# openpsi-project/srl

Hardware: AMD Instinct MI355X
Metric: env-steps/sec through GAE+PPO update, 4096 envs x 128 steps (higher is better)
Workload: dtype f32 (contractions as bf16x3 / f16x2 piece products, float32 accumulate)

## Files before the change

srl_amd/csrc/h2conv.h:

```cpp
#pragma once
#include "h2gemm.h"

namespace srlh2 {

typedef float h2_f32x4 __attribute__((ext_vector_type(4)));

enum { H2C_F2 = 0, H2C_F3 = 1, H2C_D3 = 2, H2C_D2 = 3 };
enum { H2S_LINEAR = 0, H2S_PLANAR = 1, H2S_ROWS = 2, H2S_ROWSWZ = 3 };
enum { H2D_PLANAR = 0, H2D_ROWS = 1, H2D_F32_ROUTED = 2 };

template <int ID> struct H2Geo;

template <> struct H2Geo<H2C_F2> {
  static constexpr int CGW = 1;
  static constexpr int CB = 1, NCH = 64, NTAP = 16, GW = 10, OH = 9, OW = 9, NPIX_L = 400, G = 1, PLANE_E = 400;
  static constexpr int SRC = H2S_ROWSWZ, PAD = 0, SH = 20, SW = 20, SPIX = 400;
  static constexpr int DST = H2D_PLANAR, OPIX = 81, OCH = 64;
  static constexpr bool ZERO_BORDER = false;
  static constexpr bool DENSE = false;
  __host__ __device__ static constexpr int tap_u(int t) { return (((t >> 2) & 1) * 2 + (t & 1)) * 100 + (t >> 3) * 10 + ((t & 3) >> 1); }
  __host__ __device__ static constexpr int tap_k(int t) { return t; }
};
template <> struct H2Geo<H2C_F3> {
  static constexpr int CGW = 1;
  static constexpr int CB = 2, NCH = 64, NTAP = 9, GW = 9, OH = 7, OW = 7, NPIX_L = 81, G = 2, PLANE_E = 176;
  static constexpr int SRC = H2S_PLANAR, PAD = 0, SH = 9, SW = 9, SPIX = 81;
  static constexpr int DST = H2D_ROWS, OPIX = 49, OCH = 64;
  static constexpr bool ZERO_BORDER = false;
  static constexpr bool DENSE = false;
  __host__ __device__ static constexpr int tap_u(int t) { return (t / 3) * 9 + t % 3; }
  __host__ __device__ static constexpr int tap_k(int t) { return t; }
};
template <> struct H2Geo<H2C_D3> {
  static constexpr int CGW = 1;
  static constexpr int CB = 2, NCH = 64, NTAP = 9, GW = 11, OH = 9, OW = 9, NPIX_L = 121, G = 2, PLANE_E = 256;
  static constexpr int SRC = H2S_ROWS, PAD = 2, SH = 7, SW = 7, SPIX = 49;
  static constexpr int DST = H2D_PLANAR, OPIX = 81, OCH = 64;
  static constexpr bool ZERO_BORDER = true;
  static constexpr bool DENSE = true;
  __host__ __device__ static constexpr int tap_u(int t) { return (2 - t / 3) * 11 + (2 - t % 3); }
  __host__ __device__ static constexpr int tap_k(int t) { return t; }
};
template <> struct H2Geo<H2C_D2> {
  static constexpr int CGW = 2;
  static constexpr int CB = 2, NCH = 128, NTAP = 4, GW = 11, OH = 10, OW = 10, NPIX_L = 121, G = 2, PLANE_E = 256;
  static constexpr int SRC = H2S_PLANAR, PAD = 1, SH = 9, SW = 9, SPIX = 81;
  static constexpr int DST = H2D_F32_ROUTED, OPIX = 400, OCH = 32;
  static constexpr bool ZERO_BORDER = true;
  static constexpr bool DENSE = true;
  __host__ __device__ static constexpr int tap_u(int t) { return (1 - t / 2) * 11 + (1 - t % 2); }
  __host__ __device__ static constexpr int tap_k(int t) { return t; }
};

struct H2ConvArgs {
  const void* x;
  const void* w;
  const float* sx;
  const float* sw;
  int64_t n;
  const float* bias;
  int32_t act;
  void* out;
  float* out_scale;
  const float* bound_in;
  const float* bound_w;
  const float* bound_b;
  float* out_absmax;
  uint8_t* mask_out;
  const void* mask_in;
};

#ifdef __HIPCC__

template <int ID> constexpr int h2c_src_img_bytes() { return H2Geo<ID>::SPIX * H2Geo<ID>::CB * 128; }
template <int ID> constexpr int h2c_slot_bytes() { return H2Geo<ID>::CB * 8 * H2Geo<ID>::PLANE_E * 16; }

__device__ __forceinline__ uint32_t h2_xor32(uint32_t x, bool upper) {
#if __has_builtin(__builtin_amdgcn_permlane32_swap)
  typedef unsigned h2_u32x2 __attribute__((ext_vector_type(2)));
  const h2_u32x2 r = __builtin_amdgcn_permlane32_swap(x, x, false, false);
  return upper ? r[0] : r[1];
#else
  (void)upper;
  return (uint32_t)__shfl_xor((int)x, 32);
#endif
}

#ifndef SRL_H2C_SCHED
#define SRL_H2C_SCHED 1
#endif

template <int NKB> struct H2ActiveKb { int n; int kb[NKB]; };
template <int RM, int NTAP, int CB, int TPR> constexpr H2ActiveKb<NTAP * CB> h2_active_kbs() {
  H2ActiveKb<NTAP * CB> a{};
  for (int kb = 0; kb < NTAP * CB; ++kb)
    if ((RM >> ((kb / CB) / TPR)) & 1) a.kb[a.n++] = kb;
  return a;
}

template <int ID, int NSLOT>
__global__ __launch_bounds__(512, 2) void h2conv_kernel(H2ConvArgs a) {
  using GE = H2Geo<ID>;
  constexpr int CB = GE::CB, NKB = GE::NTAP * CB, NPL = CB * 8, PLANE_B = GE::PLANE_E * 16;
  constexpr int SLOT = NPL * PLANE_B;
  constexpr int NCG = GE::NCH / 16;
  constexpr int CGW = GE::CGW, NWG = NCG / CGW;
  constexpr int NPH = 8 / NWG;
  static_assert(NWG == 4 || NWG == 8, "");
  constexpr int NE = GE::DENSE ? GE::OH * GE::OW : (GE::OH - 1) * GE::GW + GE::OW;
  constexpr int NB_IMG = (NE + 15) / 16;
  constexpr int NBT = NB_IMG * GE::G;
  static_assert(NBT % NPH == 0 && NPH <= 2, "blocks split evenly over the (at most two) position halves");
  constexpr int NDMA = SLOT / 1024;
  constexpr int NDW = (NDMA + 7) / 8;
  static_assert(SLOT % 1024 == 0, "");
  constexpr int KROW = NKB * 128;
  constexpr int IMGB = h2c_src_img_bytes<ID>();
  constexpr bool ROUTED = GE::DST == H2D_F32_ROUTED;
  constexpr int OIMGB = GE::OPIX * GE::OCH * 4;
  constexpr int MIMGB = GE::OPIX * GE::OCH / 8;
  constexpr bool MASK_IN = ID == H2C_D3 || ID == H2C_D2, MASK_OUT = !MASK_IN;
  constexpr int MREG = MASK_IN ? (GE::G * MIMGB + 1023) / 1024 * 1024 : 0;
  constexpr int SLOTM = SLOT + MREG;
  constexpr int NDM = MREG / 1024;
  extern __shared__ __attribute__((aligned(1024))) uint8_t lds[];

  const int tid = threadIdx.x, lane = tid & 63;
  const int wid = __builtin_amdgcn_readfirstlane(tid >> 6);
  const int cg0 = (wid % NWG) * CGW, ph = wid / NWG;
  const int p = lane & 15, quad = lane >> 4;
  const bool up = quad >> 1;

  h2_f16x8 wf[CGW][NKB][2];
  {
#pragma unroll
    for (int c = 0; c < CGW; ++c) {
      const uint8_t* wr = static_cast<const uint8_t*>(a.w) + (size_t)((cg0 + c) * 16 + p) * KROW + quad * 32;
#pragma unroll
      for (int kb = 0; kb < NKB; ++kb) {
        wf[c][kb][0] = *reinterpret_cast<const h2_f16x8*>(wr + kb * 128);
        wf[c][kb][1] = *reinterpret_cast<const h2_f16x8*>(wr + kb * 128 + 16);
      }
    }
#pragma unroll
    for (int c = 0; c < CGW; ++c)
#pragma unroll
      for (int kb = 0; kb < NKB; ++kb) asm volatile("" : "+v"(wf[c][kb][0]), "+v"(wf[c][kb][1]));
  }
  const float inv = 1.f / (*a.sx * *a.sw);
  float oscale = 1.f;
  if (!ROUTED) {
    float bound = *a.bound_in * *a.bound_w;
    if (a.bound_b) bound += *a.bound_b;
    oscale = h2_scale_for(bound);
    if (blockIdx.x == 0 && tid == 0) *a.out_scale = oscale;
  }
  float bq[CGW][4];
#pragma unroll
  for (int c = 0; c < CGW; ++c) {
    bq[c][0] = bq[c][1] = bq[c][2] = bq[c][3] = 0.f;
    if (a.bias) {
      const float4 b4 = *reinterpret_cast<const float4*>(a.bias + (cg0 + c) * 16 + 4 * quad);
      bq[c][0] = b4.x; bq[c][1] = b4.y; bq[c][2] = b4.z; bq[c][3] = b4.w;
    }
  }
  const float lo = a.act == 1 ? 0.f : -3.0e38f;

  if (GE::ZERO_BORDER) {
    for (int i = tid; i < NSLOT * SLOTM / 16; i += 512) reinterpret_cast<uint4*>(lds)[i] = make_uint4(0, 0, 0, 0);
    __syncthreads();
  }

  const h2_i32x4 rx = h2_rsrc(a.x);
  h2_i32x4 rmd = h2_rsrc(MASK_IN ? a.mask_in : a.x);
  rmd[2] = MASK_IN ? (int)(a.n * MIMGB) : 0;
  const uint32_t lds0 = (uint32_t)(uintptr_t)(__attribute__((address_space(3))) uint8_t*)lds;
  const long nbatch = (a.n + GE::G - 1) / GE::G;

  uint32_t dvoff[NDW];
  int dimg[NDW];
#pragma unroll
  for (int q = 0; q < NDW; ++q) {
    const int j = wid + 8 * q;
    const int nent = j * 64 + lane;
    if (GE::SRC == H2S_LINEAR) {
      dvoff[q] = (uint32_t)(nent * 16);
      dimg[q] = j < NDMA ? 0 : -1;
    } else if (GE::SRC == H2S_ROWSWZ) {
      const int P = nent >> 3, sl = nent & 7;
      dvoff[q] = (uint32_t)(P * 128 + 16 * (sl ^ (((P >> 1) & 1) | (((P >> 2) & 1) << 2))));
      dimg[q] = j < NDMA ? 0 : -1;
    } else {
      const int plane = nent / GE::PLANE_E, e = nent - plane * GE::PLANE_E;
      const int il = e / GE::NPIX_L, cell = e - il * GE::NPIX_L;
      const int gy = cell / GE::GW, gx = cell - gy * GE::GW;
      const int sy = gy - GE::PAD, sx = gx - GE::PAD;
      const bool ok = j < NDMA && il < GE::G && (unsigned)sy < (unsigned)GE::SH && (unsigned)sx < (unsigned)GE::SW;
      const int sp = sy * GE::SW + sx;
      if (GE::SRC == H2S_PLANAR) dvoff[q] = (uint32_t)(il * IMGB + plane * (GE::SPIX * 16) + sp * 16);
      else dvoff[q] = (uint32_t)((il * GE::SPIX + sp) * (CB * 128) + plane * 16);
      dimg[q] = ok ? il : -1;
      if (!ok) dvoff[q] = 0;
    }
  }
  auto issue = [&](long b, int s) {
    const long img0 = b * GE::G;
    const int left = (int)(a.n - img0 < GE::G ? a.n - img0 : GE::G);
    const uint32_t soff = __builtin_amdgcn_readfirstlane((uint32_t)(img0 * (long)IMGB));
#pragma unroll
    for (int q = 0; q < NDW; ++q) {
      const uint32_t ldsa = __builtin_amdgcn_readfirstlane(lds0 + s * SLOTM + (wid + 8 * q) * 1024);
      if (dimg[q] >= 0 && dimg[q] < left)
        asm volatile("s_mov_b32 m0, %0\n\ts_nop 4\n\tbuffer_load_dwordx4 %1, %2, %3 offen lds" ::"s"(ldsa), "v"(dvoff[q]), "s"(rx), "s"(soff) : "memory");
    }
    if (MASK_IN && wid < NDM) {
      const uint32_t ldsa = __builtin_amdgcn_readfirstlane(lds0 + s * SLOTM + SLOT + wid * 1024);
      const uint32_t msoff = __builtin_amdgcn_readfirstlane((uint32_t)(img0 * (long)MIMGB));
      const uint32_t mvoff = (uint32_t)(wid * 1024 + lane * 16);
      asm volatile("s_mov_b32 m0, %0\n\ts_nop 4\n\tbuffer_load_dwordx4 %1, %2, %3 offen lds" ::"s"(ldsa), "v"(mvoff), "s"(rmd), "s"(msoff) : "memory");
    }
  };

  uint32_t lane_out[CGW];
  uint32_t lane_mout[CGW];
  int mi_shift[CGW], mi_pix[CGW];
  int pix_step_y, pix_step_x;
#pragma unroll
  for (int c = 0; c < CGW; ++c) {
    const int cg = cg0 + c;
    const int g_out = 2 * (quad & 1) + (cg & 1), ocb = cg >> 1;
    if (ROUTED) {
      const int cls = cg >> 1, py = cls >> 1, px = cls & 1;
      lane_out[c] = (uint32_t)(((py * 20 + px) * GE::OCH + 16 * (cg & 1) + 4 * quad) * 4);
      lane_mout[c] = 0;
      mi_shift[c] = 16 * (cg & 1) + 4 * quad;
      mi_pix[c] = py * 20 + px;
    } else {
      lane_out[c] = GE::DST == H2D_PLANAR ? (uint32_t)((((ocb * 4 + g_out) * 2 + (up ? 1 : 0)) * GE::OPIX) * 16)
                                          : (uint32_t)(ocb * 128 + g_out * 32 + (up ? 16 : 0));
      lane_mout[c] = (uint32_t)(ocb * 4 + g_out);
      mi_shift[c] = 0;
      mi_pix[c] = 0;
    }
  }
  if (ROUTED) { pix_step_y = 40; pix_step_x = 2; }
  else { pix_step_y = GE::OW; pix_step_x = 1; }
  constexpr int PIXB = ROUTED ? GE::OCH * 4 : (GE::DST == H2D_PLANAR ? 16 : GE::OCH * 4);
  const uint32_t lane_base = GE::SRC == H2S_ROWSWZ ? (uint32_t)(p * 128 + quad * 32) : (uint32_t)(quad * 2 * PLANE_B + p * 16);
  int swz_d0[8], swz_d1[8];
  if (GE::SRC == H2S_ROWSWZ) {
    static_assert(GE::SRC != H2S_ROWSWZ || SLOTM % 128 == 0, "slot stride must keep address bits 4-6");
    const uint32_t a_ref = (uint32_t)(uintptr_t)(lds + lane_base);
#pragma unroll
    for (int u = 0; u < 8; ++u) {
      const int k = (p + u) & 7;
      const uint32_t x = (uint32_t)((((k >> 1) & 1) | (((k >> 2) & 1) << 2)) * 16);
      swz_d0[u] = u * 128 + (int)((a_ref ^ x) - a_ref);
      swz_d1[u] = u * 128 + (int)((a_ref ^ x ^ 16u) - a_ref);
    }
  }
  float amax = 0.f;

  struct Meta {
    uint32_t pixoff;
    bool ok;
    long img;
    uint32_t bits[CGW];
  };
  const __amdgpu_buffer_rsrc_t r_out = __builtin_amdgcn_make_buffer_rsrc(a.out, 0, (int)(a.n * OIMGB), 0x00020000);
  const __amdgpu_buffer_rsrc_t r_mo = __builtin_amdgcn_make_buffer_rsrc(MASK_OUT ? (void*)a.mask_out : a.out, 0, (int)(a.n * MIMGB), 0x00020000);
  constexpr uint32_t OOB = 0x80000000u;
  auto epilogue1 = [&](const h2_f32x4& acc, const Meta& m, const float (&bqc)[4], uint32_t lane_out_c, uint32_t lane_mout_c, uint32_t mbits) {
    float v[4];
    constexpr bool CLAMP = ID == H2C_F2 || ID == H2C_F3;
#pragma unroll
    for (int r = 0; r < 4; ++r) v[r] = CLAMP ? fmaxf(acc[r] * inv + bqc[r], lo) : acc[r] * inv + bqc[r];
    const bool ok = m.ok;
    const uint32_t img32 = (uint32_t)m.img;
    if (MASK_IN) {
#pragma unroll
      for (int r = 0; r < 4; ++r) v[r] = __uint_as_float(__float_as_uint(v[r]) & (uint32_t)__builtin_amdgcn_sbfe((int)mbits, r, 1));
    }
    {
      const float m3 = __builtin_fmaxf(__builtin_fmaxf(fabsf(v[0]), fabsf(v[1])), fabsf(v[2]));
      const float m5 = __builtin_fmaxf(__builtin_fmaxf(m3, fabsf(v[3])), amax);
      amax = m.ok ? m5 : amax;
    }
    const uint32_t ooff = ok ? m.pixoff * PIXB + lane_out_c : OOB;
    typedef uint32_t h2_u32x4 __attribute__((ext_vector_type(4)));
    if (ROUTED) {
      h2_u32x4 d = {__float_as_uint(v[0]), __float_as_uint(v[1]), __float_as_uint(v[2]), __float_as_uint(v[3])};
      __builtin_amdgcn_raw_buffer_store_b128(d, r_out, ooff + img32 * (uint32_t)OIMGB, 0, 0);
    } else {
      uint32_t h0a, h0b, h1a, h1b;
      h2_split_pair(v[0], v[1], oscale, h0a, h1a);
      h2_split_pair(v[2], v[3], oscale, h0b, h1b);
      h2_u32x4 chunk;
#if __has_builtin(__builtin_amdgcn_permlane32_swap)
      typedef unsigned h2_u32x2 __attribute__((ext_vector_type(2)));
      const h2_u32x2 sa = __builtin_amdgcn_permlane32_swap(h0a, h1a, false, false);
      const h2_u32x2 sb = __builtin_amdgcn_permlane32_swap(h0b, h1b, false, false);
      chunk[0] = sa[0]; chunk[1] = sb[0]; chunk[2] = sa[1]; chunk[3] = sb[1];
#else
      const uint32_t r0 = h2_xor32(up ? h0a : h1a, up), r1 = h2_xor32(up ? h0b : h1b, up);
      chunk[0] = up ? r0 : h0a; chunk[1] = up ? r1 : h0b; chunk[2] = up ? h1a : r0; chunk[3] = up ? h1b : r1;
#endif
      __builtin_amdgcn_raw_buffer_store_b128(chunk, r_out, ooff + img32 * (uint32_t)OIMGB, 0, 0);
      if (MASK_OUT) {
        uint32_t nib = (v[0] > 0.f ? 1u : 0u) | (v[1] > 0.f ? 2u : 0u) | (v[2] > 0.f ? 4u : 0u) | (v[3] > 0.f ? 8u : 0u);
#if __has_builtin(__builtin_amdgcn_permlane32_swap)
        const h2_u32x2 sn = __builtin_amdgcn_permlane32_swap(nib, nib, false, false);
        const uint32_t byte = sn[0] | (sn[1] << 4);
#else
        const uint32_t byte = nib | (h2_xor32(nib, up) << 4);
#endif
        const uint32_t moff = (ok && !up) ? m.pixoff * (GE::OCH / 8) + lane_mout_c : OOB;
        __builtin_amdgcn_raw_buffer_store_b8((unsigned char)byte, r_mo, moff + img32 * (uint32_t)MIMGB, 0, 0);
      }
    }
  };
  auto epilogue = [&](const h2_f32x4 (&accs)[CGW], const Meta& m) {
#pragma unroll
    for (int c = 0; c < CGW; ++c) epilogue1(accs[c], m, bq[c], lane_out[c], lane_mout[c], m.bits[c]);
  };

  constexpr int PD = CB == 1 ? 3 : (ID == H2C_D2 ? 1 : 2);
  const bool late = wid >= 4;
  auto block = [&](auto rows_c, const uint8_t* xb, h2_f32x4 (&pacc)[CGW], Meta& pm, const Meta& nm) {
    constexpr int TPR = ID == H2C_D3 ? 3 : (ID == H2C_D2 ? 2 : GE::NTAP);
    constexpr H2ActiveKb<NKB> AK = h2_active_kbs<decltype(rows_c)::value, GE::NTAP, CB, TPR>();
    h2_f32x4 acc[CGW];
#pragma unroll
    for (int c = 0; c < CGW; ++c) acc[c] = h2_f32x4{0.f, 0.f, 0.f, 0.f};
    h2_f16x8 xr[PD + 1][2];
    const uint8_t* tq0[8];
    const uint8_t* tq1[8];
    if (GE::SRC == H2S_ROWSWZ) {
#pragma unroll
      for (int u = 0; u < 8; ++u) {
        tq0[u] = xb + swz_d0[u];
        tq1[u] = xb + swz_d1[u];
      }
    }
    auto fetch = [&](int i) {
      const int kb = AK.kb[i];
      const int t = kb / CB, c = kb - t * CB;
      if (GE::SRC == H2S_ROWSWZ) {
        const int U = GE::tap_u(t), u8 = U & 7;
        xr[i % (PD + 1)][0] = *reinterpret_cast<const h2_f16x8*>(tq0[u8] + (U - u8) * 128);
        xr[i % (PD + 1)][1] = *reinterpret_cast<const h2_f16x8*>(tq1[u8] + (U - u8) * 128);
      } else {
        const int off = (c * 8) * PLANE_B + GE::tap_u(t) * 16;
        xr[i % (PD + 1)][0] = *reinterpret_cast<const h2_f16x8*>(xb + off);
        xr[i % (PD + 1)][1] = *reinterpret_cast<const h2_f16x8*>(xb + off + PLANE_B);
      }
    };
#pragma unroll
    for (int i = 0; i < PD; ++i) fetch(i);
#pragma unroll
    for (int i = 0; i < AK.n; ++i) {
      if (i + PD < AK.n) fetch(i + PD);
      if (i == 1 && !late) epilogue(pacc, pm);
      if (i == AK.n / 2 + 1 && late) epilogue(pacc, pm);
      const int kb = AK.kb[i];
      const int t = kb / CB, c = kb - t * CB;
      const int kw = GE::tap_k(t) * CB + c;
#pragma unroll
      for (int cc = 0; cc < CGW; ++cc) {
        acc[cc] = __builtin_amdgcn_mfma_f32_16x16x32_f16(wf[cc][kw][1], xr[i % (PD + 1)][0], acc[cc], 0, 0, 0);
        acc[cc] = __builtin_amdgcn_mfma_f32_16x16x32_f16(wf[cc][kw][0], xr[i % (PD + 1)][1], acc[cc], 0, 0, 0);
        acc[cc] = __builtin_amdgcn_mfma_f32_16x16x32_f16(wf[cc][kw][0], xr[i % (PD + 1)][0], acc[cc], 0, 0, 0);
      }
    }
#pragma unroll
    for (int c = 0; c < CGW; ++c) pacc[c] = acc[c];
    pm = nm;
  };

  h2_f32x4 pacc[CGW];
#pragma unroll
  for (int c = 0; c < CGW; ++c) pacc[c] = h2_f32x4{0.f, 0.f, 0.f, 0.f};
  Meta pm = {};
  pm.ok = false;
  auto compute = [&](auto phc_c, long b, int s) {
    constexpr int phc = decltype(phc_c)::value;
    const uint8_t* slot = lds + s * SLOTM + lane_base;
    const uint8_t* mreg = lds + s * SLOTM + SLOT;
#pragma unroll
    for (int jj = 0; jj < NBT / NPH; ++jj) {
      const int jb = phc * (NBT / NPH) + jj;
      const int il = jb / NB_IMG, bi = jb - il * NB_IMG;
      const int e = bi * 16 + p;
      constexpr int EW = GE::DENSE ? GE::OW : GE::GW;
      const int oy = (e * (65536 / EW + 1)) >> 16, ox = e - oy * EW;
      Meta nm;
      nm.img = b * GE::G + il;
      nm.ok = ox < GE::OW && oy < GE::OH && nm.img < a.n;
      nm.pixoff = (uint32_t)(oy * pix_step_y + ox * pix_step_x);
#pragma unroll
      for (int c = 0; c < CGW; ++c) {
        nm.bits[c] = 0u;
        if (MASK_IN) {
          const uint32_t po = nm.ok ? nm.pixoff : 0u;
          if (ID == H2C_D3) nm.bits[c] = (uint32_t)mreg[il * MIMGB + po * (GE::OCH / 8) + lane_mout[c]] >> (up ? 4 : 0);
          else nm.bits[c] = *reinterpret_cast<const uint32_t*>(mreg + il * MIMGB + (po + mi_pix[c]) * 4) >> mi_shift[c];
        }
      }
      const uint8_t* xb_ = slot + (il * GE::NPIX_L + bi * 16) * (GE::SRC == H2S_ROWSWZ ? 128 : 16) +
                           (GE::DENSE ? oy * ((GE::GW - GE::OW) * 16) : 0);
      if (ID == H2C_D3) {
        static_assert(ID != H2C_D3 || (NB_IMG == 6 && GE::GW == 11 && GE::OW == 9 && GE::NTAP == 9 && GE::SRC != H2S_ROWSWZ),
                      "row masks below are conv3's");
        if (bi == 0) block(std::integral_constant<int, 0b011>{}, xb_, pacc, pm, nm);
        else if (bi == 4) block(std::integral_constant<int, 0b110>{}, xb_, pacc, pm, nm);
        else if (bi == 5) block(std::integral_constant<int, 0b100>{}, xb_, pacc, pm, nm);
        else block(std::integral_constant<int, 0b111>{}, xb_, pacc, pm, nm);
      } else if (ID == H2C_D2) {
        static_assert(ID != H2C_D2 || (NB_IMG == 7 && GE::GW == 11 && GE::OW == 10 && GE::NTAP == 4), "row mask below is conv2's");
        if (bi == 6) block(std::integral_constant<int, 0b10>{}, xb_, pacc, pm, nm);
        else block(std::integral_constant<int, 0b11>{}, xb_, pacc, pm, nm);
      } else {
        block(std::integral_constant<int, (1 << 30) - 1>{}, xb_, pacc, pm, nm);
      }
    }
  };

  long b = blockIdx.x;
#pragma unroll
  for (int s = 0; s < NSLOT - 1; ++s)
    if (b + (long)s * gridDim.x < nbatch) issue(b + (long)s * gridDim.x, s);
  int s_cur = 0, s_nxt = NSLOT - 1;
  for (; b < nbatch; b += gridDim.x) {
    asm volatile("s_waitcnt vmcnt(0)\n\ts_waitcnt lgkmcnt(0)" ::: "memory");
    __builtin_amdgcn_s_barrier();
    const long bn = b + (long)(NSLOT - 1) * gridDim.x;
    if (bn < nbatch) issue(bn, s_nxt);
    if (ph == 0) compute(std::integral_constant<int, 0>{}, b, s_cur);
    else compute(std::integral_constant<int, NPH - 1>{}, b, s_cur);
    s_cur = s_cur + 1 == NSLOT ? 0 : s_cur + 1;
    s_nxt = s_nxt + 1 == NSLOT ? 0 : s_nxt + 1;
  }
  epilogue(pacc, pm);
  {
#pragma unroll
    for (int o = 32; o >= 1; o >>= 1) amax = fmaxf(amax, __shfl_xor(amax, o));
    if (lane == 0) {
      const float cur = __hip_atomic_load(a.out_absmax, __ATOMIC_RELAXED, __HIP_MEMORY_SCOPE_AGENT);
      if (amax > cur) atomicMax(reinterpret_cast<int*>(a.out_absmax), __float_as_int(amax));
    }
  }
}

template <int ID, int NSLOT = 2>
inline int h2conv_launch(hipStream_t st, const H2ConvArgs& a, int max_blocks = 256) {
  constexpr bool MASK_IN_L = ID == H2C_D3 || ID == H2C_D2;
  constexpr int SLOT = h2c_slot_bytes<ID>() + (MASK_IN_L ? (H2Geo<ID>::G * (H2Geo<ID>::OPIX * H2Geo<ID>::OCH / 8) + 1023) / 1024 * 1024 : 0);
  static_assert(NSLOT * SLOT <= 160 * 1024, "LDS");
  static bool attr_set = false;
  auto kern = h2conv_kernel<ID, NSLOT>;
  if (!attr_set) {
    (void)hipFuncSetAttribute(reinterpret_cast<const void*>(kern), hipFuncAttributeMaxDynamicSharedMemorySize, NSLOT * SLOT);
    attr_set = true;
  }
  const long nbatch = (a.n + H2Geo<ID>::G - 1) / H2Geo<ID>::G;
  if (nbatch <= 0) return 0;
  const long grid = nbatch < max_blocks ? nbatch : max_blocks;
  hipLaunchKernelGGL(kern, dim3((unsigned)grid), dim3(512), NSLOT * SLOT, st, a);
  return 0;
}

__host__ __device__ inline int h2_entry(int y, int x, int H, int W, int order) {
  return order == 2 ? ((y & 1) * 2 + (x & 1)) * ((H / 2) * (W / 2)) + (y >> 1) * (W / 2) + (x >> 1) : y * W + x;
}
static __global__ void h2_pack_planar_kernel(const float* __restrict__ src, int64_t n, int H, int W, int C, int order, const float* absmax,
                                      const float* scale_in, float* scale_out, uint8_t* __restrict__ dst) {
  const float scale = scale_in ? *scale_in : h2_scale_for(*absmax);
  if (scale_out && blockIdx.x == 0 && threadIdx.x == 0) *scale_out = scale;
  const int64_t ngrp = n * H * W * (C / 8);
  for (int64_t t = (int64_t)blockIdx.x * blockDim.x + threadIdx.x; t < ngrp; t += (int64_t)gridDim.x * blockDim.x) {
    const int gi = (int)(t % (C / 8));
    int64_t r = t / (C / 8);
    const int x = (int)(r % W); r /= W;
    const int y = (int)(r % H);
    const int64_t img = r / H;
    const int blk = gi >> 2, g = gi & 3;
    const float* s = src + ((img * H + y) * W + x) * C + blk * 32;
    float v[8];
#pragma unroll
    for (int j = 0; j < 8; ++j) v[j] = s[h2p_elem(g, j)];
    uint4 h0, h1;
    h2_split_pair(v[0], v[1], scale, h0.x, h1.x);
    h2_split_pair(v[2], v[3], scale, h0.y, h1.y);
    h2_split_pair(v[4], v[5], scale, h0.z, h1.z);
    h2_split_pair(v[6], v[7], scale, h0.w, h1.w);
    const int NP = H * W, e = h2_entry(y, x, H, W, order);
    uint8_t* d = dst + img * (int64_t)(NP * C * 4);
    *reinterpret_cast<uint4*>(d + ((int64_t)((blk * 4 + g) * 2 + 0) * NP + e) * 16) = h0;
    *reinterpret_cast<uint4*>(d + ((int64_t)((blk * 4 + g) * 2 + 1) * NP + e) * 16) = h1;
  }
}
static __global__ void h2_pack_pixrows_kernel(const float* __restrict__ src, int64_t n, int H, int W, int C, int order, const float* absmax,
                                       const float* scale_in, float* scale_out, uint8_t* __restrict__ dst) {
  const float scale = scale_in ? *scale_in : h2_scale_for(*absmax);
  if (scale_out && blockIdx.x == 0 && threadIdx.x == 0) *scale_out = scale;
  const int64_t ngrp = n * H * W * (C / 8);
  for (int64_t t = (int64_t)blockIdx.x * blockDim.x + threadIdx.x; t < ngrp; t += (int64_t)gridDim.x * blockDim.x) {
    const int gi = (int)(t % (C / 8));
    int64_t r = t / (C / 8);
    const int x = (int)(r % W); r /= W;
    const int y = (int)(r % H);
    const int64_t img = r / H;
    const int blk = gi >> 2, g = gi & 3;
    const float* s = src + ((img * H + y) * W + x) * C + blk * 32;
    float v[8];
#pragma unroll
    for (int j = 0; j < 8; ++j) v[j] = s[h2p_elem(g, j)];
    uint4 h0, h1;
    h2_split_pair(v[0], v[1], scale, h0.x, h1.x);
    h2_split_pair(v[2], v[3], scale, h0.y, h1.y);
    h2_split_pair(v[4], v[5], scale, h0.z, h1.z);
    h2_split_pair(v[6], v[7], scale, h0.w, h1.w);
    uint4* d = reinterpret_cast<uint4*>(dst + ((img * (int64_t)(H * W) + h2_entry(y, x, H, W, order)) * C + blk * 32) * 4 + g * 32);
    d[0] = h0;
    d[1] = h1;
  }
}
static __global__ void h2_unpack_planar_kernel(const uint8_t* __restrict__ src, int64_t n, int H, int W, int C, int order, const float* scale,
                                        float* __restrict__ dst) {
  const float inv = 1.f / *scale;
  const int64_t ngrp = n * H * W * (C / 8);
  for (int64_t t = (int64_t)blockIdx.x * blockDim.x + threadIdx.x; t < ngrp; t += (int64_t)gridDim.x * blockDim.x) {
    const int gi = (int)(t % (C / 8));
    int64_t r = t / (C / 8);
    const int x = (int)(r % W); r /= W;
    const int y = (int)(r % H);
    const int64_t img = r / H;
    const int blk = gi >> 2, g = gi & 3;
    const int NP = H * W, e = h2_entry(y, x, H, W, order);
    const uint8_t* d = src + img * (int64_t)(NP * C * 4);
    const _Float16* p0 = reinterpret_cast<const _Float16*>(d + ((int64_t)((blk * 4 + g) * 2 + 0) * NP + e) * 16);
    const _Float16* p1 = reinterpret_cast<const _Float16*>(d + ((int64_t)((blk * 4 + g) * 2 + 1) * NP + e) * 16);
    float* o = dst + ((img * H + y) * W + x) * C + blk * 32;
#pragma unroll
    for (int j = 0; j < 8; ++j) o[h2p_elem(g, j)] = ((float)p0[j] + (float)p1[j]) * inv;
  }
}

#endif

enum { H2W_C2 = 0, H2W_C3 = 1 };

template <int ID> struct H2WGeo;
template <> struct H2WGeo<H2W_C2> {
  static constexpr int CIN = 32, NTAP = 16, GW = 10, OH = 9, OW = 9, XPIX = 400, ZPIX = 81, ZW = 9;
  static constexpr bool X_ROWS = true, Z_ROWS = false;
  static constexpr int MC = 4, NN = 4;
  __host__ __device__ static constexpr int tap_u(int t) { return (((t >> 2) & 1) * 2 + (t & 1)) * 100 + (t >> 3) * 10 + ((t & 3) >> 1); }
};
template <> struct H2WGeo<H2W_C3> {
  static constexpr int CIN = 64, NTAP = 9, GW = 9, OH = 7, OW = 7, XPIX = 81, ZPIX = 49, ZW = 7;
  static constexpr bool X_ROWS = false, Z_ROWS = true;
  static constexpr int MC = 2, NN = 9;
  __host__ __device__ static constexpr int tap_u(int t) { return (t / 3) * 9 + t % 3; }
};

struct H2WgradArgs {
  const void* x;
  const void* dz;
  const float* sx;
  const float* sz;
  int64_t n;
  float* slabs;
};

#ifdef __HIPCC__

typedef short h2_s16x4 __attribute__((ext_vector_type(4)));

__host__ __device__ constexpr int h2w_plane_base(int idx, int plane) { return idx * plane + (idx >> 3) * 256 + (((idx >> 1) & 3) >= 2 ? 128 : 0); }

__device__ __forceinline__ h2_s16x4 h2_tr_read(const uint8_t* p) {
  typedef __attribute__((address_space(3))) h2_s16x4 lds_s16x4;
  return __builtin_amdgcn_ds_read_tr16_b64_v4i16((lds_s16x4*)p);
}

template <int ID, int NSLOT>
__global__ __launch_bounds__(512, 2) void h2wgrad_kernel(H2WgradArgs a) {
  using GE = H2WGeo<ID>;
  constexpr int CBX = GE::CIN / 32;
  constexpr int NE = (GE::OH - 1) * GE::GW + GE::OW;
  constexpr int NCHUNK = (NE + 31) / 32;
  constexpr int ZE = NCHUNK * 32;
  constexpr int ZPLANE = ZE * 16;
  constexpr int ZBYTES = 16 * ZPLANE + 512;
  constexpr int XE = GE::X_ROWS ? GE::XPIX : ((GE::XPIX + 15) / 16) * 16;
  constexpr int XPLANE = XE * 16;
  constexpr int XBYTES = GE::X_ROWS ? GE::XPIX * 128 : CBX * 8 * XPLANE + CBX * 256;
  constexpr int XB_AL = (XBYTES + 1023) / 1024 * 1024, ZB_AL = (ZBYTES + 1023) / 1024 * 1024;
  constexpr int SLOT = XB_AL + ZB_AL;
  constexpr int NDX = XB_AL / 1024, NDZ = ZB_AL / 1024, NDMA = NDX + NDZ, NDW = (NDMA + 7) / 8;
  constexpr int K = GE::NTAP * GE::CIN;
  constexpr int XIMGB = GE::XPIX * GE::CIN * 4, ZIMGB = GE::ZPIX * 64 * 4;
  static_assert(NSLOT * SLOT <= 160 * 1024, "LDS");
  extern __shared__ __attribute__((aligned(1024))) uint8_t lds[];

  const int tid = threadIdx.x, lane = tid & 63;
  const int wid = __builtin_amdgcn_readfirstlane(tid >> 6);
  const int o = lane >> 4, q = (lane >> 2) & 3, p = lane & 3;

  for (int i = tid; i < NSLOT * SLOT / 16; i += 512) reinterpret_cast<uint4*>(lds)[i] = make_uint4(0, 0, 0, 0);
  __syncthreads();

  const h2_i32x4 rx = h2_rsrc(a.x), rz = h2_rsrc(a.dz);
  const uint32_t lds0 = (uint32_t)(uintptr_t)(__attribute__((address_space(3))) uint8_t*)lds;
  int dvoff[NDW];
#pragma unroll
  for (int qd = 0; qd < NDW; ++qd) {
    const int j = wid + 8 * qd;
    int off = -1;
    if (j < NDX) {
      const int b = j * 1024 + lane * 16;
      if (GE::X_ROWS) {
        const int P = b >> 7, sl = (b >> 4) & 7;
        if (P < GE::XPIX) off = P * 128 + 16 * (sl ^ (((P >> 1) & 1) | (((P >> 2) & 1) << 2)));
      } else {
#pragma unroll
        for (int pl_i = 0; pl_i < CBX * 8; ++pl_i) {
          const int rel = b - h2w_plane_base(pl_i, XPLANE);
          if (rel >= 0 && rel < XPLANE && (rel >> 4) < GE::XPIX) off = pl_i * (GE::XPIX * 16) + (rel >> 4) * 16;
        }
      }
    } else if (j < NDMA) {
      const int b = (j - NDX) * 1024 + lane * 16;
#pragma unroll
      for (int pl_i = 0; pl_i < 16; ++pl_i) {
        const int rel = b - h2w_plane_base(pl_i, ZPLANE);
        if (rel >= 0 && rel < ZPLANE) {
          const int e = rel >> 4, oy = e / GE::GW, ox = e - oy * GE::GW;
          if (ox < GE::OW && oy < GE::OH) {
            const int zp = oy * GE::ZW + ox;
            off = GE::Z_ROWS ? zp * 256 + pl_i * 16 : pl_i * (GE::ZPIX * 16) + zp * 16;
          }
        }
      }
    }
    dvoff[qd] = off;
  }
  auto issue_one = [&](uint32_t sox, uint32_t soz, int s, int qd) {
    const int j = wid + 8 * qd;
    const uint32_t ldsa = __builtin_amdgcn_readfirstlane(lds0 + s * SLOT + j * 1024);
    if (dvoff[qd] >= 0) {
      if (j < NDX) asm volatile("s_mov_b32 m0, %0\n\ts_nop 4\n\tbuffer_load_dwordx4 %1, %2, %3 offen lds" ::"s"(ldsa), "v"(dvoff[qd]), "s"(rx), "s"(sox) : "memory");
      else asm volatile("s_mov_b32 m0, %0\n\ts_nop 4\n\tbuffer_load_dwordx4 %1, %2, %3 offen lds" ::"s"(ldsa), "v"(dvoff[qd]), "s"(rz), "s"(soz) : "memory");
    }
  };
  auto issue = [&](long img, int s) {
    const uint32_t sox = __builtin_amdgcn_readfirstlane((uint32_t)(img * (long)XIMGB));
    const uint32_t soz = __builtin_amdgcn_readfirstlane((uint32_t)(img * (long)ZIMGB));
#pragma unroll
    for (int qd = 0; qd < NDW; ++qd) issue_one(sox, soz, s, qd);
  };

  auto zplane = [&](int cb32, int g, int pl) { return h2w_plane_base((cb32 * 4 + g) * 2 + pl, ZPLANE); };
  const int ent = 4 * o + q, half8 = 8 * (p >> 1);
  const int mc0 = GE::MC == 4 ? 0 : (wid & 1) * 2;
  uint32_t za[GE::MC];
#pragma unroll
  for (int m = 0; m < GE::MC; ++m) {
    const int cbk = mc0 + m;
    za[m] = (uint32_t)(XB_AL + zplane(cbk >> 1, 2 * (p & 1) + (cbk & 1), 0) + ent * 16 + half8);
  }
  constexpr int CPB = GE::CIN / 16;
  constexpr int XG2 = 4 * XPLANE + 128;
  static_assert(h2w_plane_base(4, XPLANE) - h2w_plane_base(0, XPLANE) == XG2 && h2w_plane_base(7, XPLANE) - h2w_plane_base(3, XPLANE) == XG2 &&
                    h2w_plane_base(12, XPLANE) - h2w_plane_base(8, XPLANE) == XG2 && h2w_plane_base(15, XPLANE) - h2w_plane_base(11, XPLANE) == XG2,
                "x planes: lane part");
  const uint32_t xl_planar = (uint32_t)((p & 1) * XG2 + ent * 16 + half8);

  h2_f16x8 ones;
#pragma unroll
  for (int e = 0; e < 8; ++e) ones[e] = (_Float16)1.0f;

  long img = blockIdx.x;
  const long gstep = gridDim.x;
#pragma unroll
  for (int s = 0; s < NSLOT - 1; ++s)
    if (img + (long)s * gstep < a.n) issue(img + (long)s * gstep, s);

  auto run = [&](auto g_c) {
    constexpr int G = decltype(g_c)::value;
    constexpr int nn0 = G * GE::NN;
    constexpr bool MINE = GE::MC == 4 ? G < 4 : G < 1;
    constexpr int NP = NCHUNK * GE::NN;
    uint32_t xl[2][2];
#pragma unroll
    for (int t2 = 0; t2 < 2; ++t2)
#pragma unroll
      for (int pl = 0; pl < 2; ++pl) {
        if (GE::X_ROWS) {
          const int k = (ent + (GE::tap_u(nn0 / CPB + t2) & 7)) & 7;
          const uint32_t sg = (uint32_t)((((k >> 1) & 1) | (((k >> 2) & 1) << 2)) * 16);
          xl[t2][pl] = (uint32_t)(ent * 128 + half8) + (((uint32_t)(64 * (p & 1) + 16 * pl)) ^ sg);
        } else {
          xl[t2][pl] = xl_planar;
        }
      }

    h2_f32x4 acc[GE::MC][GE::NN];
#pragma unroll
    for (int m = 0; m < GE::MC; ++m)
#pragma unroll
      for (int n2 = 0; n2 < GE::NN; ++n2) acc[m][n2] = h2_f32x4{0.f, 0.f, 0.f, 0.f};
    h2_f32x4 dbacc[2] = {h2_f32x4{0.f, 0.f, 0.f, 0.f}, h2_f32x4{0.f, 0.f, 0.f, 0.f}};

    union Frag { h2_s16x4 s[2]; h2_f16x8 v; };
    constexpr int DMA_AT = (GE::MC == 4 ? G >= 4 : G >= 2) ? -1 : 48;
    static_assert(DMA_AT < NP * 3 * GE::MC, "the DMA block has a gap");
    auto image = [&](int s, bool dma, long in, int sn) {
      const uint8_t* slot = lds + s * SLOT;
      const uint32_t sox = __builtin_amdgcn_readfirstlane((uint32_t)(in * (long)XIMGB));
      const uint32_t soz = __builtin_amdgcn_readfirstlane((uint32_t)(in * (long)ZIMGB));
      auto dma_block = [&]() {
        if (dma) {
#pragma unroll
          for (int qd = 0; qd < NDW; ++qd) issue_one(sox, soz, sn, qd);
        }
      };
      if (DMA_AT < 0) dma_block();
      const uint8_t* zb[GE::MC];
#pragma unroll
      for (int m = 0; m < GE::MC; ++m) zb[m] = slot + za[m];
      const uint8_t* xb[2][2];
#pragma unroll
      for (int t2 = 0; t2 < 2; ++t2)
#pragma unroll
        for (int pl = 0; pl < 2; ++pl) xb[t2][pl] = slot + xl[t2][pl];
      Frag af[GE::MC][2], xf[2][2];
      auto rd_z = [&](int c, int m, int pl, int h) { af[m][pl].s[h] = h2_tr_read(zb[m] + pl * ZPLANE + c * 512 + h * 256); };
      auto rd_x = [&](int k, int pl, int h) {
        const int c = k / GE::NN, n2 = k - c * GE::NN;
        const int nn = nn0 + n2, tap = nn / CPB, c16x = nn - tap * CPB;
        const int U = GE::tap_u(tap);
        if constexpr (GE::X_ROWS) xf[k & 1][pl].s[h] = h2_tr_read(xb[tap - nn0 / CPB][pl] + (c * 32 + U + 16 * h) * 128 + 32 * c16x);
        else xf[k & 1][pl].s[h] = h2_tr_read(xb[0][0] + h2w_plane_base(((c16x >> 1) * 4 + (c16x & 1)) * 2 + pl, XPLANE) + (c * 32 + U) * 16 + h * 256);
      };
// ... 152 lines not shown
```

Before: 6.226 million.

## Software-pipeline conv kernel: cross-block prefetch ring, split epilogue, deferred DMA issue

Rewrites the conv kernel's inner schedule. The compute loop is now fully unrolled at compile time, and the LDS fetch ring carries across block boundaries, so the first taps of the next block are prefetched during the current one. The epilogue is split into pieces that are interleaved between MFMAs under explicit sched_barriers. The next-slot DMA issue moves from before compute to a fixed MFMA position, placed differently for early and late waves. For conv F3 it also keeps overlapping tap operands in registers across adjacent blocks to skip redundant LDS reads, at the cost of more registers and a rigid hand schedule.

```diff
diff --git a/srl_amd/csrc/h2conv.h b/srl_amd/csrc/h2conv.h
--- a/srl_amd/csrc/h2conv.h
+++ b/srl_amd/csrc/h2conv.h
@@ -86,9 +86,10 @@
 #endif
 }
 
-#ifndef SRL_H2C_SCHED
-#define SRL_H2C_SCHED 1
-#endif
+template <class F, int... I> __device__ __forceinline__ void h2_static_for_(F&& f, std::integer_sequence<int, I...>) {
+  (f(std::integral_constant<int, I>{}), ...);
+}
+template <int N, class F> __device__ __forceinline__ void h2_static_for(F&& f) { h2_static_for_(f, std::make_integer_sequence<int, N>{}); }
 
 template <int NKB> struct H2ActiveKb { int n; int kb[NKB]; };
 template <int RM, int NTAP, int CB, int TPR> constexpr H2ActiveKb<NTAP * CB> h2_active_kbs() {
@@ -96,6 +97,23 @@
   for (int kb = 0; kb < NTAP * CB; ++kb)
     if ((RM >> ((kb / CB) / TPR)) & 1) a.kb[a.n++] = kb;
   return a;
+}
+template <int ID> constexpr int h2c_tpr() { return ID == H2C_D3 ? 3 : (ID == H2C_D2 ? 2 : H2Geo<ID>::NTAP); }
+template <int ID> constexpr int h2c_row_mask(int bi) {
+  if (ID == H2C_D3) return bi == 0 ? 0b011 : (bi == 4 ? 0b110 : (bi == 5 ? 0b100 : 0b111));
+  if (ID == H2C_D2) return bi == 6 ? 0b10 : 0b11;
+  return (1 << 30) - 1;
+}
+template <int ID> constexpr int h2c_nkb(int bi) {
+  int n = 0;
+  for (int kb = 0; kb < H2Geo<ID>::NTAP * H2Geo<ID>::CB; ++kb)
+    if ((h2c_row_mask<ID>(bi) >> ((kb / H2Geo<ID>::CB) / h2c_tpr<ID>())) & 1) ++n;
+  return n;
+}
+template <int ID> constexpr int h2c_kbs_before(int jb0, int jj, int nb_img) {
+  int g = 0;
+  for (int k = 0; k < jj; ++k) g += h2c_nkb<ID>((jb0 + k) % nb_img);
+  return g;
 }
 
 template <int ID, int NSLOT>
@@ -262,140 +280,102 @@
   float amax = 0.f;
 
   struct Meta {
+    long img;
     uint32_t pixoff;
-    bool ok;
-    long img;
-    uint32_t bits[CGW];
+    uint32_t ok;
+    uint32_t bits[2];
   };
+  static_assert(CGW <= 2 && sizeof(Meta) == 24, "");
   const __amdgpu_buffer_rsrc_t r_out = __builtin_amdgcn_make_buffer_rsrc(a.out, 0, (int)(a.n * OIMGB), 0x00020000);
   const __amdgpu_buffer_rsrc_t r_mo = __builtin_amdgcn_make_buffer_rsrc(MASK_OUT ? (void*)a.mask_out : a.out, 0, (int)(a.n * MIMGB), 0x00020000);
   constexpr uint32_t OOB = 0x80000000u;
-  auto epilogue1 = [&](const h2_f32x4& acc, const Meta& m, const float (&bqc)[4], uint32_t lane_out_c, uint32_t lane_mout_c, uint32_t mbits) {
-    float v[4];
-    constexpr bool CLAMP = ID == H2C_F2 || ID == H2C_F3;
-#pragma unroll
-    for (int r = 0; r < 4; ++r) v[r] = CLAMP ? fmaxf(acc[r] * inv + bqc[r], lo) : acc[r] * inv + bqc[r];
+  constexpr int EPP = MASK_OUT ? 3 : 2;
+  constexpr int NEP = CGW * EPP;
+  float ev[CGW][4];
+#pragma unroll
+  for (int c = 0; c < CGW; ++c) ev[c][0] = ev[c][1] = ev[c][2] = ev[c][3] = 0.f;
+  auto epi_piece = [&](int k, const h2_f32x4 (&accs)[CGW], const Meta& m) {
+    const int c = k / EPP, q = k - c * EPP;
+    float (&v)[4] = ev[c];
     const bool ok = m.ok;
     const uint32_t img32 = (uint32_t)m.img;
-    if (MASK_IN) {
-#pragma unroll
-      for (int r = 0; r < 4; ++r) v[r] = __uint_as_float(__float_as_uint(v[r]) & (uint32_t)__builtin_amdgcn_sbfe((int)mbits, r, 1));
-    }
-    {
+    typedef uint32_t h2_u32x4 __attribute__((ext_vector_type(4)));
+#if __has_builtin(__builtin_amdgcn_permlane32_swap)
+    typedef unsigned h2_u32x2 __attribute__((ext_vector_type(2)));
+#endif
+    if (q == 0) {
+      constexpr bool CLAMP = ID == H2C_F2 || ID == H2C_F3;
+#pragma unroll
+      for (int r = 0; r < 4; ++r) v[r] = CLAMP ? fmaxf(accs[c][r] * inv + bq[c][r], lo) : accs[c][r] * inv + bq[c][r];
+      if (MASK_IN) {
+#pragma unroll
+        for (int r = 0; r < 4; ++r) v[r] = __uint_as_float(__float_as_uint(v[r]) & (uint32_t)__builtin_amdgcn_sbfe((int)m.bits[c], r, 1));
+      }
       const float m3 = __builtin_fmaxf(__builtin_fmaxf(fabsf(v[0]), fabsf(v[1])), fabsf(v[2]));
       const float m5 = __builtin_fmaxf(__builtin_fmaxf(m3, fabsf(v[3])), amax);
       amax = m.ok ? m5 : amax;
-    }
-    const uint32_t ooff = ok ? m.pixoff * PIXB + lane_out_c : OOB;
-    typedef uint32_t h2_u32x4 __attribute__((ext_vector_type(4)));
-    if (ROUTED) {
-      h2_u32x4 d = {__float_as_uint(v[0]), __float_as_uint(v[1]), __float_as_uint(v[2]), __float_as_uint(v[3])};
-      __builtin_amdgcn_raw_buffer_store_b128(d, r_out, ooff + img32 * (uint32_t)OIMGB, 0, 0);
+    } else if (q == 1) {
+      const uint32_t ooff = ok ? m.pixoff * PIXB + lane_out[c] : OOB;
+      if (ROUTED) {
+        h2_u32x4 d = {__float_as_uint(v[0]), __float_as_uint(v[1]), __float_as_uint(v[2]), __float_as_uint(v[3])};
+        __builtin_amdgcn_raw_buffer_store_b128(d, r_out, ooff + img32 * (uint32_t)OIMGB, 0, 0);
+      } else {
+        uint32_t h0a, h0b, h1a, h1b;
+        h2_split_pair(v[0], v[1], oscale, h0a, h1a);
+        h2_split_pair(v[2], v[3], oscale, h0b, h1b);
+        h2_u32x4 chunk;
+#if __has_builtin(__builtin_amdgcn_permlane32_swap)
+        const h2_u32x2 sa = __builtin_amdgcn_permlane32_swap(h0a, h1a, false, false);
+        const h2_u32x2 sb = __builtin_amdgcn_permlane32_swap(h0b, h1b, false, false);
+        chunk[0] = sa[0]; chunk[1] = sb[0]; chunk[2] = sa[1]; chunk[3] = sb[1];
+#else
+        const uint32_t r0 = h2_xor32(up ? h0a : h1a, up), r1 = h2_xor32(up ? h0b : h1b, up);
+        chunk[0] = up ? r0 : h0a; chunk[1] = up ? r1 : h0b; chunk[2] = up ? h1a : r0; chunk[3] = up ? h1b : r1;
+#endif
+        __builtin_amdgcn_raw_buffer_store_b128(chunk, r_out, ooff + img32 * (uint32_t)OIMGB, 0, 0);
+      }
     } else {
-      uint32_t h0a, h0b, h1a, h1b;
-      h2_split_pair(v[0], v[1], oscale, h0a, h1a);
-      h2_split_pair(v[2], v[3], oscale, h0b, h1b);
-      h2_u32x4 chunk;
+      uint32_t nib = (v[0] > 0.f ? 1u : 0u) | (v[1] > 0.f ? 2u : 0u) | (v[2] > 0.f ? 4u : 0u) | (v[3] > 0.f ? 8u : 0u);
 #if __has_builtin(__builtin_amdgcn_permlane32_swap)
-      typedef unsigned h2_u32x2 __attribute__((ext_vector_type(2)));
-      const h2_u32x2 sa = __builtin_amdgcn_permlane32_swap(h0a, h1a, false, false);
-      const h2_u32x2 sb = __builtin_amdgcn_permlane32_swap(h0b, h1b, false, false);
-      chunk[0] = sa[0]; chunk[1] = sb[0]; chunk[2] = sa[1]; chunk[3] = sb[1];
+      const h2_u32x2 sn = __builtin_amdgcn_permlane32_swap(nib, nib, false, false);
+      const uint32_t byte = sn[0] | (sn[1] << 4);
 #else
-      const uint32_t r0 = h2_xor32(up ? h0a : h1a, up), r1 = h2_xor32(up ? h0b : h1b, up);
-      chunk[0] = up ? r0 : h0a; chunk[1] = up ? r1 : h0b; chunk[2] = up ? h1a : r0; chunk[3] = up ? h1b : r1;
+      const uint32_t byte = nib | (h2_xor32(nib, up) << 4);
 #endif
-      __builtin_amdgcn_raw_buffer_store_b128(chunk, r_out, ooff + img32 * (uint32_t)OIMGB, 0, 0);
-      if (MASK_OUT) {
-        uint32_t nib = (v[0] > 0.f ? 1u : 0u) | (v[1] > 0.f ? 2u : 0u) | (v[2] > 0.f ? 4u : 0u) | (v[3] > 0.f ? 8u : 0u);
-#if __has_builtin(__builtin_amdgcn_permlane32_swap)
-        const h2_u32x2 sn = __builtin_amdgcn_permlane32_swap(nib, nib, false, false);
-        const uint32_t byte = sn[0] | (sn[1] << 4);
-#else
-        const uint32_t byte = nib | (h2_xor32(nib, up) << 4);
-#endif
-        const uint32_t moff = (ok && !up) ? m.pixoff * (GE::OCH / 8) + lane_mout_c : OOB;
-        __builtin_amdgcn_raw_buffer_store_b8((unsigned char)byte, r_mo, moff + img32 * (uint32_t)MIMGB, 0, 0);
-      }
+      const uint32_t moff = (ok && !up) ? m.pixoff * (GE::OCH / 8) + lane_mout[c] : OOB;
+      __builtin_amdgcn_raw_buffer_store_b8((unsigned char)byte, r_mo, moff + img32 * (uint32_t)MIMGB, 0, 0);
     }
   };
-  auto epilogue = [&](const h2_f32x4 (&accs)[CGW], const Meta& m) {
-#pragma unroll
-    for (int c = 0; c < CGW; ++c) epilogue1(accs[c], m, bq[c], lane_out[c], lane_mout[c], m.bits[c]);
-  };
 
   constexpr int PD = CB == 1 ? 3 : (ID == H2C_D2 ? 1 : 2);
+  constexpr int TPR = h2c_tpr<ID>();
+  static_assert(ID != H2C_D3 || (NB_IMG == 6 && GE::GW == 11 && GE::OW == 9 && GE::NTAP == 9 && GE::SRC != H2S_ROWSWZ), "h2c_row_mask: conv3's");
+  static_assert(ID != H2C_D2 || (NB_IMG == 7 && GE::GW == 11 && GE::OW == 10 && GE::NTAP == 4), "h2c_row_mask: conv2's");
+  static_assert(GE::SRC != H2S_ROWSWZ || (GE::G == 1 && ((NB_IMG - 1) * 16 + GE::tap_u(GE::NTAP - 1) + 8) * 128 < 65536), "table register + immediate");
   const bool late = wid >= 4;
-  auto block = [&](auto rows_c, const uint8_t* xb, h2_f32x4 (&pacc)[CGW], Meta& pm, const Meta& nm) {
-    constexpr int TPR = ID == H2C_D3 ? 3 : (ID == H2C_D2 ? 2 : GE::NTAP);
-    constexpr H2ActiveKb<NKB> AK = h2_active_kbs<decltype(rows_c)::value, GE::NTAP, CB, TPR>();
-    h2_f32x4 acc[CGW];
-#pragma unroll
-    for (int c = 0; c < CGW; ++c) acc[c] = h2_f32x4{0.f, 0.f, 0.f, 0.f};
-    h2_f16x8 xr[PD + 1][2];
-    const uint8_t* tq0[8];
-    const uint8_t* tq1[8];
-    if (GE::SRC == H2S_ROWSWZ) {
-#pragma unroll
-      for (int u = 0; u < 8; ++u) {
-        tq0[u] = xb + swz_d0[u];
-        tq1[u] = xb + swz_d1[u];
-      }
-    }
-    auto fetch = [&](int i) {
-      const int kb = AK.kb[i];
-      const int t = kb / CB, c = kb - t * CB;
-      if (GE::SRC == H2S_ROWSWZ) {
-        const int U = GE::tap_u(t), u8 = U & 7;
-        xr[i % (PD + 1)][0] = *reinterpret_cast<const h2_f16x8*>(tq0[u8] + (U - u8) * 128);
-        xr[i % (PD + 1)][1] = *reinterpret_cast<const h2_f16x8*>(tq1[u8] + (U - u8) * 128);
-      } else {
-        const int off = (c * 8) * PLANE_B + GE::tap_u(t) * 16;
-        xr[i % (PD + 1)][0] = *reinterpret_cast<const h2_f16x8*>(xb + off);
-        xr[i % (PD + 1)][1] = *reinterpret_cast<const h2_f16x8*>(xb + off + PLANE_B);
-      }
-    };
-#pragma unroll
-    for (int i = 0; i < PD; ++i) fetch(i);
-#pragma unroll
-    for (int i = 0; i < AK.n; ++i) {
-      if (i + PD < AK.n) fetch(i + PD);
-      if (i == 1 && !late) epilogue(pacc, pm);
-      if (i == AK.n / 2 + 1 && late) epilogue(pacc, pm);
-      const int kb = AK.kb[i];
-      const int t = kb / CB, c = kb - t * CB;
-      const int kw = GE::tap_k(t) * CB + c;
-#pragma unroll
-      for (int cc = 0; cc < CGW; ++cc) {
-        acc[cc] = __builtin_amdgcn_mfma_f32_16x16x32_f16(wf[cc][kw][1], xr[i % (PD + 1)][0], acc[cc], 0, 0, 0);
-        acc[cc] = __builtin_amdgcn_mfma_f32_16x16x32_f16(wf[cc][kw][0], xr[i % (PD + 1)][1], acc[cc], 0, 0, 0);
-        acc[cc] = __builtin_amdgcn_mfma_f32_16x16x32_f16(wf[cc][kw][0], xr[i % (PD + 1)][0], acc[cc], 0, 0, 0);
-      }
-    }
-#pragma unroll
-    for (int c = 0; c < CGW; ++c) pacc[c] = acc[c];
-    pm = nm;
-  };
+  constexpr bool DMA_HOLD_LATE = ID == H2C_F2;
+  constexpr int DMA_AT = ID == H2C_F2 || ID == H2C_F3 ? 16 : 24;
 
   h2_f32x4 pacc[CGW];
 #pragma unroll
   for (int c = 0; c < CGW; ++c) pacc[c] = h2_f32x4{0.f, 0.f, 0.f, 0.f};
   Meta pm = {};
-  pm.ok = false;
-  auto compute = [&](auto phc_c, long b, int s) {
+  pm.ok = 0u;
+  auto compute = [&](auto phc_c, long b, int s, long bn, int sn) {
     constexpr int phc = decltype(phc_c)::value;
+    constexpr int NJ = NBT / NPH;
+    constexpr int ESZ = GE::SRC == H2S_ROWSWZ ? 128 : 16;
     const uint8_t* slot = lds + s * SLOTM + lane_base;
     const uint8_t* mreg = lds + s * SLOTM + SLOT;
-#pragma unroll
-    for (int jj = 0; jj < NBT / NPH; ++jj) {
-      const int jb = phc * (NBT / NPH) + jj;
-      const int il = jb / NB_IMG, bi = jb - il * NB_IMG;
+    constexpr int EW = GE::DENSE ? GE::OW : GE::GW;
+    auto oy_of = [&](int bi) { return ((bi * 16 + p) * (65536 / EW + 1)) >> 16; };
+    auto meta_of = [&](int il, int bi) {
       const int e = bi * 16 + p;
-      constexpr int EW = GE::DENSE ? GE::OW : GE::GW;
-      const int oy = (e * (65536 / EW + 1)) >> 16, ox = e - oy * EW;
+      const int oy = oy_of(bi), ox = e - oy * EW;
       Meta nm;
       nm.img = b * GE::G + il;
-      nm.ok = ox < GE::OW && oy < GE::OH && nm.img < a.n;
+      nm.ok = ox < GE::OW && oy < GE::OH && nm.img < a.n ? 1u : 0u;
+      nm.bits[0] = nm.bits[1] = 0u;
       nm.pixoff = (uint32_t)(oy * pix_step_y + ox * pix_step_x);
 #pragma unroll
       for (int c = 0; c < CGW; ++c) {
@@ -406,41 +386,141 @@
           else nm.bits[c] = *reinterpret_cast<const uint32_t*>(mreg + il * MIMGB + (po + mi_pix[c]) * 4) >> mi_shift[c];
         }
       }
-      const uint8_t* xb_ = slot + (il * GE::NPIX_L + bi * 16) * (GE::SRC == H2S_ROWSWZ ? 128 : 16) +
-                           (GE::DENSE ? oy * ((GE::GW - GE::OW) * 16) : 0);
-      if (ID == H2C_D3) {
-        static_assert(ID != H2C_D3 || (NB_IMG == 6 && GE::GW == 11 && GE::OW == 9 && GE::NTAP == 9 && GE::SRC != H2S_ROWSWZ),
-                      "row masks below are conv3's");
-        if (bi == 0) block(std::integral_constant<int, 0b011>{}, xb_, pacc, pm, nm);
-        else if (bi == 4) block(std::integral_constant<int, 0b110>{}, xb_, pacc, pm, nm);
-        else if (bi == 5) block(std::integral_constant<int, 0b100>{}, xb_, pacc, pm, nm);
-        else block(std::integral_constant<int, 0b111>{}, xb_, pacc, pm, nm);
-      } else if (ID == H2C_D2) {
-        static_assert(ID != H2C_D2 || (NB_IMG == 7 && GE::GW == 11 && GE::OW == 10 && GE::NTAP == 4), "row mask below is conv2's");
-        if (bi == 6) block(std::integral_constant<int, 0b10>{}, xb_, pacc, pm, nm);
-        else block(std::integral_constant<int, 0b11>{}, xb_, pacc, pm, nm);
+      return nm;
+    };
+    auto xbase_of = [&](int bi) -> const uint8_t* { return GE::DENSE ? slot + oy_of(bi) * ((GE::GW - GE::OW) * 16) : slot; };
+    const uint8_t* tq0[8];
+    const uint8_t* tq1[8];
+    if (GE::SRC == H2S_ROWSWZ) {
+#pragma unroll
+      for (int u = 0; u < 8; ++u) {
+        tq0[u] = slot + swz_d0[u];
+        tq1[u] = slot + swz_d1[u];
+      }
+    }
+    h2_f16x8 xr[PD + 1][2];
+    constexpr bool KEEP = ID == H2C_F3;
+    constexpr int KEEP_OUT_T = 6, KEEP_IN_T = 2;
+    static_assert(!KEEP || (GE::tap_u(KEEP_OUT_T) == 16 + GE::tap_u(KEEP_IN_T) && KEEP_OUT_T * CB - PD > KEEP_IN_T * CB + CB - 1 && KEEP_IN_T * CB >= PD),
+                  "kept taps: same entries, re-read only behind their second use, never part of a burst");
+    h2_f16x8 xk[CB][2];
+    auto fetch = [&](int kb, int r, int h, const uint8_t* xb, int boff, bool has_pred, bool has_succ) {
+      const int t = kb / CB, c = kb - t * CB;
+      if (KEEP && has_pred && t == KEEP_IN_T) return;
+      if (KEEP && has_succ && t == KEEP_OUT_T) {
+        xk[c][h] = *reinterpret_cast<const h2_f16x8*>(xb + boff + (c * 8 + h) * PLANE_B + GE::tap_u(t) * 16);
+        return;
+      }
+      if (GE::SRC == H2S_ROWSWZ) {
+        const int U = GE::tap_u(t), u8 = U & 7;
+        if (h == 0) xr[r][0] = *reinterpret_cast<const h2_f16x8*>(tq0[u8] + boff + (U - u8) * 128);
+        else xr[r][1] = *reinterpret_cast<const h2_f16x8*>(tq1[u8] + boff + (U - u8) * 128);
       } else {
-        block(std::integral_constant<int, (1 << 30) - 1>{}, xb_, pacc, pm, nm);
-      }
-    }
+        xr[r][h] = *reinterpret_cast<const h2_f16x8*>(xb + boff + (c * 8 + h) * PLANE_B + GE::tap_u(t) * 16);
+      }
+    };
+
+    const bool dma = bn < nbatch;
+    if (dma && late != DMA_HOLD_LATE) issue(bn, sn);
+    const uint8_t* xbc = xbase_of((phc * NJ) % NB_IMG);
+    {
+      constexpr int il0 = (phc * NJ) / NB_IMG, bi0 = (phc * NJ) % NB_IMG;
+      constexpr H2ActiveKb<NKB> AK0 = h2_active_kbs<h2c_row_mask<ID>(bi0), GE::NTAP, CB, TPR>();
+#pragma unroll
+      for (int i = 0; i < PD; ++i) {
+        fetch(AK0.kb[i], i, 0, xbc, (il0 * GE::NPIX_L + bi0 * 16) * ESZ, false, false);
+        fetch(AK0.kb[i], i, 1, xbc, (il0 * GE::NPIX_L + bi0 * 16) * ESZ, false, false);
+      }
+    }
+    __builtin_amdgcn_sched_barrier(0);
+    h2_static_for<NJ>([&](auto jj_c) {
+      constexpr int jj = decltype(jj_c)::value;
+      constexpr int jb = phc * NJ + jj, il = jb / NB_IMG, bi = jb - il * NB_IMG;
+      constexpr bool LASTB = jj + 1 == NJ;
+      constexpr int jbn = LASTB ? jb : jb + 1, iln = jbn / NB_IMG, bin = jbn - iln * NB_IMG;
+      constexpr H2ActiveKb<NKB> AK = h2_active_kbs<h2c_row_mask<ID>(bi), GE::NTAP, CB, TPR>();
+      constexpr H2ActiveKb<NKB> AKN = h2_active_kbs<h2c_row_mask<ID>(bin), GE::NTAP, CB, TPR>();
+      constexpr int N = AK.n, NT = N * CGW;
+      static_assert(N >= PD + 1 && AKN.n >= PD, "the ring reaches one block ahead at most");
+      constexpr int G0 = h2c_kbs_before<ID>(phc * NJ, jj, NB_IMG);
+      constexpr int boff = (il * GE::NPIX_L + bi * 16) * ESZ, boffn = (iln * GE::NPIX_L + bin * 16) * ESZ;
+      constexpr int E_EARLY = CGW, E_LATE = (N / 2 + 1) * CGW;
+      constexpr int XN_AT = (N - PD - 1) * CGW;
+      constexpr int META_AT = NT - 2;
+      constexpr bool HAS_PRED = KEEP && jj > 0 && bi > 0, HAS_SUCC = KEEP && !LASTB && iln == il && bin == bi + 1;
+      h2_f32x4 acc[CGW];
+#pragma unroll
+      for (int c = 0; c < CGW; ++c) acc[c] = h2_f32x4{0.f, 0.f, 0.f, 0.f};
+      const uint8_t* xbn = xbc;
+      Meta nm = pm;
+#pragma unroll
+      for (int i = 0; i < N; ++i) {
+        const int kb = AK.kb[i];
+        const int t = kb / CB, c = kb - t * CB;
+        const int kw = GE::tap_k(t) * CB + c;
+        const int r = (G0 + i) % (PD + 1);
+        const int ip = i + PD, rp = (G0 + ip) % (PD + 1);
+        const bool pf_here = ip < N, pf_next = ip >= N && !LASTB;
+        const bool kept = (HAS_PRED && t == KEEP_IN_T) || (HAS_SUCC && t == KEEP_OUT_T);
+        const h2_f16x8& x0 = kept ? xk[c][0] : xr[r][0];
+        const h2_f16x8& x1 = kept ? xk[c][1] : xr[r][1];
+#pragma unroll
+        for (int cc = 0; cc < CGW; ++cc) {
+          const int T = i * CGW + cc;
+          acc[cc] = __builtin_amdgcn_mfma_f32_16x16x32_f16(wf[cc][kw][1], x0, acc[cc], 0, 0, 0);
+          if (cc == 0) {
+            if (pf_here) fetch(AK.kb[ip], rp, 0, xbc, boff, HAS_PRED, HAS_SUCC);
+            else if (pf_next) fetch(AKN.kb[ip - N], rp, 0, xbn, boffn, false, false);
+          }
+          __builtin_amdgcn_sched_barrier(0);
+          acc[cc] = __builtin_amdgcn_mfma_f32_16x16x32_f16(wf[cc][kw][0], x1, acc[cc], 0, 0, 0);
+          if (cc == 0) {
+            if (pf_here) fetch(AK.kb[ip], rp, 1, xbc, boff, HAS_PRED, HAS_SUCC);
+            else if (pf_next) fetch(AKN.kb[ip - N], rp, 1, xbn, boffn, false, false);
+          }
+          __builtin_amdgcn_sched_barrier(0);
+          acc[cc] = __builtin_amdgcn_mfma_f32_16x16x32_f16(wf[cc][kw][0], x0, acc[cc], 0, 0, 0);
+          if (T == XN_AT && !LASTB && GE::DENSE) xbn = xbase_of(bin);
+          if (T == META_AT) nm = meta_of(il, bi);
+          if (T >= E_EARLY && T - E_EARLY < NEP && !late) {
+#pragma unroll
+            for (int k = T - E_EARLY; k < (T == NT - 1 ? NEP : T - E_EARLY + 1); ++k) epi_piece(k, pacc, pm);
+          }
+          if (T >= E_LATE && T - E_LATE < NEP && late) {
+#pragma unroll
+            for (int k = T - E_LATE; k < (T == NT - 1 ? NEP : T - E_LATE + 1); ++k) epi_piece(k, pacc, pm);
+          }
+          __builtin_amdgcn_sched_barrier(0);
+          if (G0 * CGW + T == DMA_AT) {
+            if (dma && late == DMA_HOLD_LATE) issue(bn, sn);
+            __builtin_amdgcn_sched_barrier(0);
+          }
+        }
+      }
+#pragma unroll
+      for (int c = 0; c < CGW; ++c) pacc[c] = acc[c];
+      pm = nm;
+      xbc = xbn;
+    });
   };
 
   long b = blockIdx.x;
+  const long gstep = gridDim.x;
 #pragma unroll
   for (int s = 0; s < NSLOT - 1; ++s)
-    if (b + (long)s * gridDim.x < nbatch) issue(b + (long)s * gridDim.x, s);
+    if (b + (long)s * gstep < nbatch) issue(b + (long)s * gstep, s);
   int s_cur = 0, s_nxt = NSLOT - 1;
-  for (; b < nbatch; b += gridDim.x) {
+  for (; b < nbatch; b += gstep) {
     asm volatile("s_waitcnt vmcnt(0)\n\ts_waitcnt lgkmcnt(0)" ::: "memory");
     __builtin_amdgcn_s_barrier();
-    const long bn = b + (long)(NSLOT - 1) * gridDim.x;
-    if (bn < nbatch) issue(bn, s_nxt);
-    if (ph == 0) compute(std::integral_constant<int, 0>{}, b, s_cur);
-    else compute(std::integral_constant<int, NPH - 1>{}, b, s_cur);
+    const long bn = b + (long)(NSLOT - 1) * gstep;
+    if (ph == 0) compute(std::integral_constant<int, 0>{}, b, s_cur, bn, s_nxt);
+    else compute(std::integral_constant<int, NPH - 1>{}, b, s_cur, bn, s_nxt);
     s_cur = s_cur + 1 == NSLOT ? 0 : s_cur + 1;
     s_nxt = s_nxt + 1 == NSLOT ? 0 : s_nxt + 1;
   }
-  epilogue(pacc, pm);
+#pragma unroll
+  for (int k = 0; k < NEP; ++k) epi_piece(k, pacc, pm);
   {
 #pragma unroll
     for (int o = 32; o >= 1; o >>= 1) amax = fmaxf(amax, __shfl_xor(amax, o));
```

Measured after the change: 6.350 million, median of 6. +2.0%, better.
